# kupc25648/MOP-truss-MARL

Hardware: AMD Instinct MI355X
Metric: env steps/sec (batched FEM solves) at 4096 envs (higher is better)
Workload: dtype f64; 1 GPU; synthetic random-geometry 2-row trusses, 32 nodes / 80 elements / 60 DOF, FEM-only env.step (action decode + FP64 assembly/solve + stresses + point), no agent; envs_per_gpu=4096, global_envs=4096, nodes=32, elements=80, ndof=60, half_bandwidth=7, lanes_per_env=16, rows_per_lane=1, parallelism=env-batch sharded over 1 GPU(s), no data-path collective

## Files before the change

mop-truss-marl_amd/csrc/truss_body.h:

```cpp
#pragma once
#include <stdint.h>
#include <math.h>

#ifndef TB_OPAQUE
#define TB_OPAQUE(x) (x)
#endif
#ifndef TB_SCHED_FENCE
#define TB_SCHED_FENCE()
#endif
#ifndef TRUSS_HD
#error "define TRUSS_HD (e.g. __device__ __forceinline__) before including truss_body.h"
#endif

#define TF_TOP 1
#define TF_RESX 2
#define TF_RESY 4
#define TF_LOAD_BRIDGE 8
#define TF_LOAD_ROOF 16

#define TB_NO_DECODE 0x1u
#define TB_CLAMP_INPLACE 0x2u
#define TB_EMIT_OBS 0x4u

#if defined(__clang__)
typedef uint32_t tb_u4 __attribute__((ext_vector_type(4)));
typedef uint32_t tb_u2 __attribute__((ext_vector_type(2)));
typedef float tb_f4 __attribute__((ext_vector_type(4)));
typedef float tb_f2 __attribute__((ext_vector_type(2)));
typedef double tb_d2 __attribute__((ext_vector_type(2)));
#else
typedef uint32_t tb_u4 __attribute__((vector_size(16)));
typedef uint32_t tb_u2 __attribute__((vector_size(8)));
typedef float tb_f4 __attribute__((vector_size(16)));
typedef float tb_f2 __attribute__((vector_size(8)));
typedef double tb_d2 __attribute__((vector_size(16)));
#endif
TRUSS_HD void tb_ld_row(const double *p, double *dst, int n2) {
  const tb_d2 *q = (const tb_d2 *)__builtin_assume_aligned(p, 16);
  for (int i = 0; i < n2; ++i) {
    tb_d2 v = q[i];
    dst[2 * i] = v[0];
    dst[2 * i + 1] = v[1];
  }
}

struct TopoDev {
  int32_t N, E, NP, ndof, n_pad, n_rest, n_sym_nodes, n_sym_elems, n_sections, has_pairs;
  int32_t nteams, KA, mid, rowsA, rowsB, zlen, dlen, zslot;
  const char *blob;
  int32_t blob_bytes;
  int32_t f_conn;
  int32_t f_pairs;
  int32_t f_nflags;
  int32_t f_dofpos;
  int32_t f_restslot;
  int32_t f_asm;
  int32_t f_diagoff;
  int32_t f_zcode;
  int32_t f_posnode;
  int32_t f_symn;
  int32_t f_syme;
  int32_t f_area;
  int32_t f_isr;
  int32_t f_adj8;
  int32_t f_exs;
  int32_t f_areaf;
  int32_t f_vsf;
  double e_mod, long_stress;
  int32_t o_env0, env_stride;
  int32_t o_kb, o_zs, o_xsol, o_red, o_rbuf, o_par, o_y, o_x, o_tg, o_geo, o_tac, o_sec, o_ev, o_zring, o_mrg;
  int32_t so_q0, so_sr, so_disp, so_mu, so_md, so_comp;
  int32_t emit_ok;
  const char *etab;
  int32_t o_flag;
  int32_t et_xn, et_nxn, et_mat, f_tnxe;
  int32_t nc_xn, nc_nxn, nc_nxe, nc_mat;
  int32_t nxe_cw;
  int32_t b_const;
  int32_t b_erec;
  int32_t b_erec2;
  int32_t b_tc;
  int32_t b_nraw;
  int32_t b_nna, b_nnb, b_nn8;
};

#define TB_TAB(type, base, off) ((const type *)((base) + (off)))

struct StepArgsDev {
  int32_t B;
  uint32_t flags;
  const float *x, *y_in;
  const int32_t *sec_in;
  const float *mu_in, *md_in;
  float *a_geo, *a_topo;
  const uint8_t *coin;
  const float *target;
  const double *env_params;
  float *y_out;
  int32_t *sec_out;
  float *mu_out, *md_out;
  float *disp, *q0, *sr;
  uint8_t *comp;
  float *point, *obj;
  double *disp64, *q064, *energy, *react;
  int32_t *status;
  float *x_n, *A_s, *A_ts, *A_cs, *nxn, *nxe;
};

#define TRUSS_NRED 6

#ifndef TRUSS_BAND_PAD
#define TRUSS_BAND_PAD 1
#endif
constexpr bool tb_band_padded(int G, int WL, int RPL, int EPL, bool emit) {
  return TRUSS_BAND_PAD == 2 ? !emit : TRUSS_BAND_PAD != 0 && !emit && G == 16 && WL == 8 && RPL == 1 && EPL == 5;
}
constexpr int tb_band_stride(int G, int WL, int RPL, int EPL, bool emit) {
  return WL * RPL + (tb_band_padded(G, WL, RPL, EPL, emit) ? 2 : 0);
}
constexpr int tb_band_team_b(int rowsA, int ks, int w) {
  return rowsA * ks + (ks != w ? ((64 - rowsA * ks * 8) & 127) / 8 : 0);
}

TRUSS_HD float tb_clamp01(float v) { return v > 1.0f ? 1.0f : (v < 0.0f ? 0.0f : v); }

TRUSS_HD float tb_round2(float v) { return rintf(v * 100.0f) / 100.0f; }

template <int G, int WL, int RPL, int EPL, bool EMIT = false>
struct StepLane {
  static constexpr int W = WL * RPL;
  static constexpr int KS = tb_band_stride(G, WL, RPL, EPL, EMIT);
  static_assert(KS % 2 == 0, "band rows are read as 16-byte units");
  static constexpr int WL_ = WL;
  static constexpr int G_ = G;
  static constexpr bool EMIT_ = EMIT;
  static constexpr int NPL = (2 * EPL + 4) / 5;
  static constexpr int EPB = 64 / G;
  static constexpr int NDEG = 8;
  static constexpr int NT = G / WL;

  int lane, g, gs, team, env, envc;
  double *Kt, *Zt, *ZRt;
  bool active;
  const char *TB;
  char *L;
  double max_def, load_x, load_y;
  float ymax32, dmin32, ymd32, int1, int2;
  int is_roof;
  double ek[EPL], ec[EPL], es[EPL], ei[EPL];
  double R[RPL][W];
  double rhs[RPL];
  double xs[W];
  int bad;
  double p_vol, p_dt, p_en;
  float p_c1, p_c2;

  TRUSS_HD double *kb(const TopoDev &T) { return (double *)(L + T.o_kb); }
  TRUSS_HD static int team_b(const TopoDev &T) { return tb_band_team_b(T.rowsA, KS, W); }
  TRUSS_HD double *zs(const TopoDev &T) { return (double *)(L + T.o_zs); }
  TRUSS_HD double *xsol(const TopoDev &T) { return (double *)(L + T.o_xsol); }
  TRUSS_HD double *red(const TopoDev &T) { return (double *)(L + T.o_red); }
  TRUSS_HD double *rbuf(const TopoDev &T) { return (double *)(L + T.o_rbuf); }
  TRUSS_HD double *par(const TopoDev &T) { return (double *)(L + T.o_par); }
  TRUSS_HD float *ysh(const TopoDev &T) { return (float *)(L + T.o_y); }
  TRUSS_HD float *xsh(const TopoDev &T) { return (float *)(L + T.o_x); }
  TRUSS_HD float *tgsh(const TopoDev &T) { return (float *)(L + T.o_tg); }
  TRUSS_HD float *geosh(const TopoDev &T) { return (float *)(L + T.o_geo); }
  TRUSS_HD float *tac(const TopoDev &T) { return (float *)(L + T.o_tac); }
  TRUSS_HD int32_t *secsh(const TopoDev &T) { return (int32_t *)(L + T.o_sec); }
  TRUSS_HD int32_t *coinsh(const TopoDev &T) { return (int32_t *)(L + T.env_stride - 4); }
  TRUSS_HD static bool coin_used(const TopoDev &T, const StepArgsDev &A) {
    return T.n_sym_nodes > 0 && !(A.flags & TB_NO_DECODE) && A.coin;
  }
  TRUSS_HD double *evsh(const TopoDev &T) { return (double *)(L + T.o_ev); }
  TRUSS_HD const int16_t *t_conn(const TopoDev &T) const { return TB_TAB(int16_t, TB, T.f_conn); }
  TRUSS_HD const int16_t *t_pairs(const TopoDev &T) const { return TB_TAB(int16_t, TB, T.f_pairs); }
  TRUSS_HD const uint8_t *t_nflags(const TopoDev &T) const { return TB_TAB(uint8_t, TB, T.f_nflags); }
  TRUSS_HD const int16_t *t_dofpos(const TopoDev &T) const { return TB_TAB(int16_t, TB, T.f_dofpos); }
  TRUSS_HD const int16_t *t_restslot(const TopoDev &T) const { return TB_TAB(int16_t, TB, T.f_restslot); }
  TRUSS_HD const int16_t *t_asm(const TopoDev &T) const { return TB_TAB(int16_t, TB, T.f_asm); }
  TRUSS_HD const int16_t *t_diagoff(const TopoDev &T) const { return TB_TAB(int16_t, TB, T.f_diagoff); }
  TRUSS_HD const uint8_t *t_zcode(const TopoDev &T) const { return TB_TAB(uint8_t, TB, T.f_zcode); }
  TRUSS_HD const int16_t *t_posnode(const TopoDev &T) const { return TB_TAB(int16_t, TB, T.f_posnode); }
  TRUSS_HD const int16_t *t_symn(const TopoDev &T) const { return TB_TAB(int16_t, TB, T.f_symn); }
  TRUSS_HD const int16_t *t_syme(const TopoDev &T) const { return TB_TAB(int16_t, TB, T.f_syme); }
  TRUSS_HD const double *t_area(const TopoDev &T) const { return TB_TAB(double, TB, T.f_area); }
  TRUSS_HD const double *t_isr(const TopoDev &T) const { return TB_TAB(double, TB, T.f_isr); }
  TRUSS_HD const int16_t *t_adj8(const TopoDev &T) const { return TB_TAB(int16_t, TB, T.f_adj8); }
  TRUSS_HD const int16_t *t_exs(const TopoDev &T) const { return TB_TAB(int16_t, TB, T.f_exs); }

  TRUSS_HD void init(int lane_, int block, const TopoDev &T, const StepArgsDev &A, char *lds) {
    lane = lane_;
    g = lane % G;
    gs = g % WL;
    team = T.nteams == 2 ? (g / WL) & 1 : 0;
    int grp = lane / G;
    env = block * EPB + grp;
    active = env < A.B;
    envc = active ? env : A.B - 1;
    TB = lds;
    L = lds + T.o_env0 + (size_t)grp * T.env_stride;
    Kt = (double *)(L + T.o_kb) + team * team_b(T);
    Zt = (double *)(L + T.o_zs) + team * T.zlen;
    ZRt = (double *)(L + T.o_zring) + team * W;
    bad = 0;
    p_vol = p_dt = p_en = 0.0;
    p_c1 = p_c2 = 0.0f;
    rs_first_step = 0;
    rs_y_out = A.y_out;
    rs_sec_out = A.sec_out;
    rs_next_geo = rs_next_topo = nullptr;
  }

  static constexpr int BIT = 8;
  static constexpr int BIT_BIG = 20;
  static constexpr int NCAP = (G * ((2 * EPL + 4) / 5) > 64) ? G * ((2 * EPL + 4) / 5) : 64;
  static constexpr int ECAP = (G * EPL > 128) ? G * EPL : 128;
  static constexpr int NIT = (NCAP / 4 + G - 1) / G;
  static constexpr int EIT = (ECAP / 4 + G - 1) / G;
  tb_u4 pg[2 * NIT], pa[3 * NIT];
  int rs_first_step;
  float *rs_y_out;
  int32_t *rs_sec_out;
  const float *rs_next_geo, *rs_next_topo;
  TRUSS_HD void rollout_prefetch(const TopoDev &T, const StepArgsDev &A) {
    if (rs_next_geo) {
      const size_t bn = (size_t)envc * T.N;
      row_load<2 * NIT>(rs_next_geo + bn * 2, 2 * (T.N >> 2), pg);
      row_load<3 * NIT>(rs_next_topo + bn * 3, 3 * (T.N >> 2), pa);
    }
  }
  TRUSS_HD void rollout_stash(const TopoDev &T, const StepArgsDev &A) {
    if (rs_next_geo) {
      row_store<2 * NIT>(geosh(T), 2 * (T.N >> 2), pg);
      row_store<3 * NIT>(tac(T), 3 * (T.N >> 2), pa);
    }
  }

  TRUSS_HD void stage_row_slow(const void *src, void *dst, int nwords) const {
    const uint32_t *s1 = (const uint32_t *)src;
    uint32_t *d1 = (uint32_t *)dst;
    for (int q = g; q < nwords; q += G) d1[q] = s1[q];
  }

  template <int IT>
  TRUSS_HD void row_load(const void *src, int nq, tb_u4 (&v)[IT]) const {
    const tb_u4 *s4 = (const tb_u4 *)src;
#pragma unroll
    for (int i = 0; i < IT; ++i) {
      int q = g + G * i;
      v[i] = s4[q < nq ? q : nq - 1];
    }
  }
  template <int IT>
  TRUSS_HD void row_store(void *dst, int nq, const tb_u4 (&v)[IT]) const {
    tb_u4 *d4 = (tb_u4 *)dst;
#pragma unroll
    for (int i = 0; i < IT; ++i) {
      int q = g + G * i;
      d4[q < nq ? q : nq - 1] = v[i];
    }
  }

  TRUSS_HD void band_clear(const TopoDev &T) {
    tb_u4 *K4 = (tb_u4 *)kb(T);
    const tb_u4 z = {0u, 0u, 0u, 0u};
    const int tot4 = (KS == W ? (T.rowsA + T.rowsB) * W : team_b(T) + T.rowsB * KS) >> 1;
    for (int i = g; i < tot4; i += G) K4[i] = z;
  }

  template <int BI>
  TRUSS_HD void stage_fast(const TopoDev &T, const StepArgsDev &A, bool decode) {
    const size_t bn = (size_t)envc * T.N, be = (size_t)envc * T.E;
    {
      const int nb = T.blob_bytes >> 4, nn = T.N >> 2, ne = T.E >> 2;
      tb_u4 vb[BI], vy[NIT], vx[NIT], vt[NIT], vs[EIT], vp[1], vg[2 * NIT], va[3 * NIT];
      {
        const tb_u4 *s4 = (const tb_u4 *)T.blob;
#pragma unroll
        for (int i = 0; i < BI; ++i) {
          int q = lane + 64 * i;
          vb[i] = s4[q < nb ? q : nb - 1];
        }
      }
      row_load<NIT>(A.y_in + bn, nn, vy);
      row_load<NIT>(A.x + bn, nn, vx);
      row_load<NIT>(A.target + bn, nn, vt);
      row_load<EIT>(A.sec_in + be, ne, vs);
      row_load<1>(A.env_params + (size_t)envc * 8, 4, vp);
      if (decode) {
        row_load<2 * NIT>(A.a_geo + bn * 2, 2 * nn, vg);
        row_load<3 * NIT>(A.a_topo + bn * 3, 3 * nn, va);
      }
      const bool coin = coin_used(T, A);
      int cb = 0;
      if (coin) cb = A.coin[envc];
      band_clear(T);
      {
        tb_u4 *d4 = (tb_u4 *)TB;
#pragma unroll
        for (int i = 0; i < BI; ++i) {
          int q = lane + 64 * i;
          d4[q < nb ? q : nb - 1] = vb[i];
        }
      }
      row_store<NIT>(ysh(T), nn, vy);
      row_store<NIT>(xsh(T), nn, vx);
      row_store<NIT>(tgsh(T), nn, vt);
      row_store<EIT>(secsh(T), ne, vs);
      row_store<1>(par(T), 4, vp);
      if (decode) {
        row_store<2 * NIT>(geosh(T), 2 * nn, vg);
        row_store<3 * NIT>(tac(T), 3 * nn, va);
      }
      if (coin) *coinsh(T) = cb;
    }
  }

  TRUSS_HD void phase_stage(const TopoDev &T, const StepArgsDev &A) {
    const size_t bn = (size_t)envc * T.N, be = (size_t)envc * T.E;
    const bool decode = !(A.flags & TB_NO_DECODE);
    const bool fast = (T.N & 3) == 0 && (T.E & 3) == 0 && T.N <= NCAP && T.E <= ECAP && T.blob_bytes <= BIT_BIG * 64 * 16;
    if (rs_first_step != 0) {
      band_clear(T);
      return;
    }
    if (fast) {
      if (T.blob_bytes <= 3 * 64 * 16) stage_fast<3>(T, A, decode);
      else if (T.blob_bytes <= BIT * 64 * 16) stage_fast<BIT>(T, A, decode);
      else stage_fast<BIT_BIG>(T, A, decode);
    } else {
      const bool coin = coin_used(T, A);
      int cb = 0;
      if (coin) cb = A.coin[envc];
      {
        const tb_u4 *s4 = (const tb_u4 *)T.blob;
        tb_u4 *d4 = (tb_u4 *)TB;
        for (int q = lane; q < (T.blob_bytes >> 4); q += 64) d4[q] = s4[q];
      }
      stage_row_slow(A.y_in + bn, ysh(T), T.N);
      stage_row_slow(A.x + bn, xsh(T), T.N);
      stage_row_slow(A.target + bn, tgsh(T), T.N);
      stage_row_slow(A.sec_in + be, secsh(T), T.E);
      stage_row_slow(A.env_params + (size_t)envc * 8, par(T), 16);
      if (decode) {
        stage_row_slow(A.a_geo + bn * 2, geosh(T), 2 * T.N);
        stage_row_slow(A.a_topo + bn * 3, tac(T), 3 * T.N);
      }
      band_clear(T);
      if (coin) *coinsh(T) = cb;
    }
  }

  TRUSS_HD void load_params(const TopoDev &T) {
    const double *P = par(T);
    double y_max = P[0], d_min = P[1];
    max_def = P[2];
    load_x = P[3];
    load_y = P[4];
    int1 = (float)P[5];
    int2 = (float)P[6];
    is_roof = P[7] != 0.0;
    ymax32 = (float)y_max;
    dmin32 = (float)d_min;
    ymd32 = (float)(y_max - d_min);
  }

  TRUSS_HD void move_range(bool top, float y, float yp, float &up, float &dn) const {
    float upt = fabsf(ymax32 - y), dnt = fabsf((y - yp) - dmin32);
    float upb = is_roof ? fabsf((yp - y) - dmin32) : 0.0f, dnb = is_roof ? fabsf(y) : 0.0f;
    up = top ? upt : upb;
    dn = top ? dnt : dnb;
  }

  TRUSS_HD float move_node(float y, float g0, float g1, float mu, float md, bool resy) const {
    bool down = g1 > g0;
    float a = down ? g1 : g0;
    float rng = down ? md : mu;
    float step = (a * rng) * 0.25f;
    y = down ? (y - step) : (y + step);
    y = tb_round2(y);
    return resy ? 0.0f : y;
  }

  struct PairIn {
    int n0, n1, f0, f1;
    float y0, y1, ga0, ga1, gb0, gb1, ta[3], tb[3];
    float mu0, md0, mu1, md1;
  };
  TRUSS_HD void pair_load(const TopoDev &T, int p, PairIn &q) {
    const float *Y = ysh(T), *GE = geosh(T), *TA = tac(T);
    const int16_t *PR = t_pairs(T);
    const uint8_t *NF = t_nflags(T);
    q.n0 = PR[2 * p];
    q.n1 = PR[2 * p + 1];
    q.y0 = Y[q.n0];
    q.y1 = Y[q.n1];
    q.f0 = NF[q.n0];
    q.f1 = NF[q.n1];
    q.ga0 = GE[2 * q.n0];
    q.ga1 = GE[2 * q.n0 + 1];
    q.gb0 = GE[2 * q.n1];
    q.gb1 = GE[2 * q.n1 + 1];
#pragma unroll
    for (int j = 0; j < 3; ++j) {
      q.ta[j] = TA[3 * q.n0 + j];
      q.tb[j] = TA[3 * q.n1 + j];
    }
  }
  TRUSS_HD void pair_ranges_load(const TopoDev &T, const StepArgsDev &A, PairIn &q) const {
    const size_t bn = (size_t)envc * T.N;
    q.mu0 = A.mu_in[bn + q.n0];
    q.md0 = A.md_in[bn + q.n0];
    q.mu1 = A.mu_in[bn + q.n1];
    q.md1 = A.md_in[bn + q.n1];
  }
  TRUSS_HD void pair_decode(const TopoDev &T, const StepArgsDev &A, PairIn &q, bool real) {
    const size_t bn = (size_t)envc * T.N;
    float *Y = ysh(T), *TA = tac(T);
    const int n0 = q.n0, n1 = q.n1;
    const bool top0 = q.f0 & TF_TOP, top1 = q.f1 & TF_TOP;
    const float ga0 = tb_clamp01(q.ga0), ga1 = tb_clamp01(q.ga1), gb0 = tb_clamp01(q.gb0), gb1 = tb_clamp01(q.gb1);
#pragma unroll
    for (int j = 0; j < 3; ++j) {
      q.ta[j] = tb_clamp01(q.ta[j]);
      q.tb[j] = tb_clamp01(q.tb[j]);
      TA[3 * n0 + j] = q.ta[j];
      TA[3 * n1 + j] = q.tb[j];
    }
    if ((A.flags & TB_CLAMP_INPLACE) && active && real) {
      A.a_geo[(bn + n0) * 2 + 0] = ga0;
      A.a_geo[(bn + n0) * 2 + 1] = ga1;
      A.a_geo[(bn + n1) * 2 + 0] = gb0;
      A.a_geo[(bn + n1) * 2 + 1] = gb1;
#pragma unroll
      for (int j = 0; j < 3; ++j) {
        A.a_topo[(bn + n0) * 3 + j] = q.ta[j];
        A.a_topo[(bn + n1) * 3 + j] = q.tb[j];
      }
    }
    float mu0, md0, mu1, md1;
    if (A.mu_in) {
      mu0 = q.mu0;
      md0 = q.md0;
      mu1 = q.mu1;
      md1 = q.md1;
    } else {
      move_range(top0, q.y0, q.y1, mu0, md0);
      move_range(top1, q.y1, q.y0, mu1, md1);
    }
    float a = move_node(q.y0, ga0, ga1, mu0, md0, q.f0 & TF_RESY);
    float b = move_node(q.y1, gb0, gb1, mu1, md1, q.f1 & TF_RESY);
    const bool c1 = a < 0.0f;
    a = c1 ? (top0 ? dmin32 : 0.0f) : a;
    b = (c1 && top0) ? 0.0f : b;
    const bool c2 = b < 0.0f;
    b = c2 ? (top1 ? dmin32 : 0.0f) : b;
    a = (c2 && top1) ? 0.0f : a;
    const bool c3 = a > ymax32;
    a = c3 ? (top0 ? ymax32 : ymd32) : a;
    b = (c3 && !top0) ? ymax32 : b;
    const bool c4 = b > ymax32;
    b = c4 ? (top1 ? ymax32 : ymd32) : b;
    a = (c4 && !top1) ? ymax32 : a;
    a = (top0 && fabsf(a - b) < dmin32) ? b + dmin32 : a;
    b = (top1 && fabsf(b - a) < dmin32) ? a + dmin32 : b;
    if (real) {
      Y[n0] = a;
      Y[n1] = b;
    }
  }
  TRUSS_HD void phase_decode(const TopoDev &T, const StepArgsDev &A) {
    load_params(T);
    if (A.flags & TB_NO_DECODE) return;
    constexpr int PPL = (NPL + 1) / 2;
    PairIn q[PPL];
#pragma unroll
    for (int i = 0; i < PPL; ++i) {
      const int p = g + G * i;
      pair_load(T, p < T.NP ? p : T.NP - 1, q[i]);
    }
    if (A.mu_in) {
#pragma unroll
      for (int i = 0; i < PPL; ++i) pair_ranges_load(T, A, q[i]);
    }
#pragma unroll
    for (int i = 0; i < PPL; ++i) pair_decode(T, A, q[i], g + G * i < T.NP);
    for (int p = g + G * PPL; p < T.NP; p += G) {
      PairIn r;
      pair_load(T, p, r);
      if (A.mu_in) pair_ranges_load(T, A, r);
      pair_decode(T, A, r, true);
    }
  }

  TRUSS_HD void phase_sym_nodes(const TopoDev &T) {
    float *Y = ysh(T);
    const int16_t *SN = t_symn(T);
    const bool heads = *coinsh(T) != 0;
    for (int i = g; i < T.n_sym_nodes; i += G) {
      int dst = SN[2 * i], src = SN[2 * i + 1];
      float v = heads ? Y[src] : Y[dst];
      Y[dst] = v;
      Y[src] = v;
    }
  }

  TRUSS_HD void phase_sizing(const TopoDev &T, const StepArgsDev &A) {
    if (A.flags & TB_NO_DECODE) return;
    const float *TA = tac(T);
    int32_t *S = secsh(T);
    const int16_t *CN = t_conn(T);
    int n0[EPL], n1[EPL], sc[EPL];
    float a0[EPL][3], a1[EPL][3];
#pragma unroll
    for (int i = 0; i < EPL; ++i) {
      const int e = g + G * i;
      const int ee = e < T.E ? e : T.E - 1;
      const uint32_t c = *(const uint32_t *)(CN + 2 * ee);
      n0[i] = (int)(int16_t)(c & 0xffffu);
      n1[i] = (int)(int16_t)(c >> 16);
      sc[i] = S[ee];
    }
#pragma unroll
    for (int i = 0; i < EPL; ++i) {
#pragma unroll
      for (int j = 0; j < 3; ++j) {
        a0[i][j] = TA[n0[i] * 3 + j];
        a1[i][j] = TA[n1[i] * 3 + j];
      }
    }
#pragma unroll
    for (int i = 0; i < EPL; ++i) {
      const float p0 = a0[i][0] + a1[i][0], p1 = a0[i][1] + a1[i][1], p2 = a0[i][2] + a1[i][2];
      int am = 0;
      float best = p0;
      if (p1 > best) { am = 1; best = p1; }
      if (p2 > best) { am = 2; }
      const int s = sc[i];
      const int sdn = s > 0 ? s - 1 : 0, sup = s < T.n_sections - 1 ? s + 1 : T.n_sections - 1;
      sc[i] = am == 0 ? sdn : (am == 1 ? sup : s);
    }
#pragma unroll
    for (int i = 0; i < EPL; ++i) {
      const int e = g + G * i;
      if (e < T.E) S[e] = sc[i];
    }
  }

  TRUSS_HD void phase_sym_elems(const TopoDev &T) {
    int32_t *S = secsh(T);
    const int16_t *SE = t_syme(T);
    for (int i = g; i < T.n_sym_elems; i += G) {
      int a = SE[2 * i], b = SE[2 * i + 1];
      int m = S[a] < S[b] ? S[a] : S[b];
      S[a] = m;
      S[b] = m;
    }
  }

  TRUSS_HD double load_at(const TopoDev &T, int r) const {
    if (r < 0 || r >= T.ndof) return 0.0;
    int nd = t_posnode(T)[r];
    if (nd < 0) return 0.0;
    int fl = t_nflags(T)[nd >> 1] & (is_roof ? TF_LOAD_ROOF : TF_LOAD_BRIDGE);
    if (!fl) return 0.0;
    return (nd & 1) ? load_y : load_x;
  }
  TRUSS_HD int orig_pos(const TopoDev &T, int tm, int p) const { return tm ? T.ndof - 1 - p : p; }
  TRUSS_HD double team_load(const TopoDev &T, int tm, int p) const {
    if (T.nteams == 1) return load_at(T, p);
    if (tm == 0) return p < T.ndof - T.KA ? load_at(T, p) : 0.0;
    return p < T.KA ? load_at(T, T.ndof - 1 - p) : 0.0;
  }

  static constexpr bool EBATCH = RPL == 1 && W <= 8 && EPL <= 5;
  static constexpr int ECH = EBATCH ? EPL : 1;
  TRUSS_HD void phase_elements(const TopoDev &T, const StepArgsDev &A) {
    const float *Y = ysh(T), *X = xsh(T);
    const int32_t *S = secsh(T);
    const int16_t *CN = t_conn(T);
    const double *AR = t_area(T), *ISR = t_isr(T);
    double *K = kb(T);
    const int16_t *AC = t_asm(T);
    double *EV = evsh(T);
    if (g == 0) EV[3 * T.E] = EV[3 * T.E + 1] = EV[3 * T.E + 2] = 0.0;
#pragma unroll
    for (int c0 = 0; c0 < EPL; c0 += ECH) {
      int n0[ECH], n1[ECH], sc[ECH], ev[ECH];
      tb_u2 code[ECH];
      float x0[ECH], x1[ECH], y0[ECH], y1[ECH];
      double Aa[ECH];
#pragma unroll
      for (int j = 0; j < ECH; ++j) {
        const int i = c0 + j < EPL ? c0 + j : EPL - 1;
        const int e = g + G * i;
        const int ee = e < T.E ? e : T.E - 1;
        const uint32_t c = *(const uint32_t *)(CN + 2 * ee);
        n0[j] = (int)(int16_t)(c & 0xffffu);
        n1[j] = (int)(int16_t)(c >> 16);
        sc[j] = S[ee];
        code[j] = *(const tb_u2 *)(AC + 4 * ee);
        ev[j] = 3 * ee;
      }
#pragma unroll
      for (int j = 0; j < ECH; ++j) {
        x0[j] = X[n0[j]];
        x1[j] = X[n1[j]];
        y0[j] = Y[n0[j]];
        y1[j] = Y[n1[j]];
        Aa[j] = AR[sc[j]];
      }
#pragma unroll
      for (int j = 0; j < ECH; ++j) {
        const int i = c0 + j;
        if (i < EPL) {
          const double dx = (double)x1[j] - (double)x0[j];
          const double dy = (double)y1[j] - (double)y0[j];
          const double l2 = dx * dx + dy * dy;
          const double rl = tb_rsqrt(l2);
          const double len = l2 * rl;
          const double c = dx * rl, s = dy * rl;
// ... 1278 lines not shown
```

mop-truss-marl_amd/csrc/truss_hip.hip:

```cpp
#include <hip/hip_runtime.h>

#include <atomic>
#include <cstdint>
#include <cstdio>
#include <cstring>
#include <type_traits>

#include "../../include/truss_mi355.h"

#pragma clang fp contract(off)

#define TRUSS_HD __device__ __forceinline__
#define TRUSS_UNROLL _Pragma("unroll")
#define TB_SCHED_FENCE() __builtin_amdgcn_sched_barrier(0)
__device__ __forceinline__ int tb_opaque(int x) {
  asm volatile("" : "+v"(x));
  return x;
}
#define TB_OPAQUE(x) tb_opaque(x)
#define TB_STREAM_STORE(p, v) __builtin_nontemporal_store((v), (p))
#ifdef TRUSS_OBS_STORE_NT
#define TB_OBS_STORE(p, v) __builtin_nontemporal_store((v), (p))
#else
#define TB_OBS_STORE(p, v) (*(p) = (v))
#endif

__device__ __forceinline__ void tb_lds_add(double *p, double v) { unsafeAtomicAdd(p, v); }

template <int WL, int SRC>
__device__ __forceinline__ double tb_dpp_bcast(double v) {
#ifndef TRUSS_BCAST32
  if constexpr (WL == 16 || WL == 8) {
    const long long b = __double_as_longlong(v);
    long long r;
    if constexpr (WL == 16) {
      r = __builtin_amdgcn_update_dpp(0ll, b, 0x150 + SRC, 0xf, 0xf, false);
    } else {
      r = __builtin_amdgcn_update_dpp(0ll, b, 0x150 + SRC, 0xf, 0x3, false);
      r = __builtin_amdgcn_update_dpp(r, b, 0x150 + 8 + SRC, 0xf, 0xc, false);
    }
    return __longlong_as_double(r);
  }
#endif
  const int lo = __double2loint(v), hi = __double2hiint(v);
  int rlo, rhi;
  if constexpr (WL == 16) {
    rlo = __builtin_amdgcn_update_dpp(lo, lo, 0x150 + SRC, 0xf, 0xf, false);
    rhi = __builtin_amdgcn_update_dpp(hi, hi, 0x150 + SRC, 0xf, 0xf, false);
  } else if constexpr (WL == 8) {
    rlo = __builtin_amdgcn_update_dpp(lo, lo, 0x150 + SRC, 0xf, 0x3, false);
    rlo = __builtin_amdgcn_update_dpp(rlo, lo, 0x150 + 8 + SRC, 0xf, 0xc, false);
    rhi = __builtin_amdgcn_update_dpp(hi, hi, 0x150 + SRC, 0xf, 0x3, false);
    rhi = __builtin_amdgcn_update_dpp(rhi, hi, 0x150 + 8 + SRC, 0xf, 0xc, false);
  } else {
    static_assert(WL == 4, "team width");
    constexpr int qp = SRC | (SRC << 2) | (SRC << 4) | (SRC << 6);
    rlo = __builtin_amdgcn_update_dpp(lo, lo, qp, 0xf, 0xf, false);
    rhi = __builtin_amdgcn_update_dpp(hi, hi, qp, 0xf, 0xf, false);
  }
  return __hiloint2double(rhi, rlo);
}
template <class LN>
__device__ __forceinline__ double tb_team_bcast(LN &ln, int src) {
  constexpr int WL = LN::WL_;
  switch (src) {
#define TB_CASE(i) \
  case i:          \
    if constexpr (i < WL) return tb_dpp_bcast<WL, i>(ln.bx); else break;
    TB_CASE(0) TB_CASE(1) TB_CASE(2) TB_CASE(3) TB_CASE(4) TB_CASE(5) TB_CASE(6) TB_CASE(7)
    TB_CASE(8) TB_CASE(9) TB_CASE(10) TB_CASE(11) TB_CASE(12) TB_CASE(13) TB_CASE(14) TB_CASE(15)
#undef TB_CASE
  }
  return ln.bx;
}

__device__ __forceinline__ double tb_rcp(double d) {
  double r = __builtin_amdgcn_rcp(d);
  r = fma(fma(-d, r, 1.0), r, r);
  r = fma(fma(-d, r, 1.0), r, r);
  return r;
}

__device__ __forceinline__ float tb_rcpf(float d) {
  float r = __builtin_amdgcn_rcpf(d);
  return fmaf(fmaf(-d, r, 1.0f), r, r);
}

#ifdef TRUSS_STOP_AT
#define TRUSS_ST(i) do { if ((i) == TRUSS_STOP_AT) return; } while (0)
#endif
#ifdef TRUSS_STAMPS
__device__ unsigned long long g_truss_stamps[32];
__device__ unsigned long long g_truss_span[4096][6];
#define TRUSS_ST(i)                                                  \
  do {                                                               \
    __builtin_amdgcn_sched_barrier(0);                               \
    if (threadIdx.x == 0 && blockIdx.x == gridDim.x / 2) g_truss_stamps[i] = clock64(); \
    if (threadIdx.x == 0 && ((i) == 0 || (i) == 9) && blockIdx.x < 4096) {              \
      g_truss_span[blockIdx.x][(i) == 0 ? 0 : 2] = clock64();                            \
      g_truss_span[blockIdx.x][(i) == 0 ? 1 : 3] = wall_clock64();                       \
    }                                                                \
    __builtin_amdgcn_sched_barrier(0);                               \
  } while (0)
#endif

__device__ __forceinline__ double tb_rsqrt(double x) {
  double r = __builtin_amdgcn_rsq(x);
  r = r * fma(-0.5 * x, r * r, 1.5);
  r = r * fma(-0.5 * x, r * r, 1.5);
  return r;
}

template <int G, bool MAX>
__device__ __forceinline__ float tb_group_reduce(float v) {
  auto op = [](float a, float b) { return MAX ? fmaxf(a, b) : fminf(a, b); };
  auto dpp = [](float x, auto ctrl) {
    return __int_as_float(__builtin_amdgcn_update_dpp(0, __float_as_int(x), decltype(ctrl)::value, 0xf, 0xf, false));
  };
  if constexpr (G >= 2) v = op(v, dpp(v, std::integral_constant<int, 0xB1>{}));
  if constexpr (G >= 4) v = op(v, dpp(v, std::integral_constant<int, 0x4E>{}));
  if constexpr (G >= 8) v = op(v, dpp(v, std::integral_constant<int, 0x141>{}));
  if constexpr (G >= 16) v = op(v, dpp(v, std::integral_constant<int, 0x140>{}));
  if constexpr (G >= 32) v = op(v, __shfl_xor(v, 16));
  if constexpr (G >= 64) v = op(v, __shfl_xor(v, 32));
  return v;
}
template <class LN>
__device__ __forceinline__ float tb_group_min(LN &ln, int c) { return tb_group_reduce<LN::G_, false>(ln.pmn[c]); }
template <class LN>
__device__ __forceinline__ float tb_group_max(LN &ln, int c) { return tb_group_reduce<LN::G_, true>(ln.pmx[c]); }

template <int G>
__device__ __forceinline__ double tb_group_reduce_sum(double v) {
  auto dpp = [](double x, auto ctrl) {
    const int lo = __builtin_amdgcn_update_dpp(0, __double2loint(x), decltype(ctrl)::value, 0xf, 0xf, false);
    const int hi = __builtin_amdgcn_update_dpp(0, __double2hiint(x), decltype(ctrl)::value, 0xf, 0xf, false);
    return __hiloint2double(hi, lo);
  };
  if constexpr (G >= 2) v = v + dpp(v, std::integral_constant<int, 0xB1>{});
  if constexpr (G >= 4) v = v + dpp(v, std::integral_constant<int, 0x4E>{});
  if constexpr (G >= 8) v = v + dpp(v, std::integral_constant<int, 0x141>{});
  if constexpr (G >= 16) v = v + dpp(v, std::integral_constant<int, 0x140>{});
  if constexpr (G >= 32) v = v + __shfl_xor(v, 16);
  if constexpr (G >= 64) v = v + __shfl_xor(v, 32);
  return v;
}
template <class LN>
__device__ __forceinline__ double tb_group_sum_d(LN &ln, int which) {
  return tb_group_reduce_sum<LN::G_>(which == 0 ? ln.p_vol : which == 1 ? ln.p_dt : ln.p_en);
}
template <class LN>
__device__ __forceinline__ float tb_group_max_f(LN &ln, int which) {
  return tb_group_reduce<LN::G_, true>(which == 0 ? ln.p_c1 : which == 1 ? ln.p_c2 : (float)ln.bad);
}

template <class LN, class TD>
__device__ __forceinline__ bool tb_obs_timed_out(LN &ln, const TD &T) {
  if constexpr (LN::EMIT_) return *((const __attribute__((address_space(3))) int *)(ln.TB + T.o_flag) + 1) != 0;
  return false;
}

#include "truss_body.h"

typedef __attribute__((address_space(3))) int tb_lds_word;
__device__ __forceinline__ tb_lds_word *tb_flag_ptr(char *lds, int o_flag) { return (tb_lds_word *)(lds + o_flag); }
__device__ __forceinline__ void tb_publish(char *lds, int o_flag, int k) {
  __builtin_amdgcn_wave_barrier();
#ifdef TRUSS_FLAG_RELAXED
  __builtin_amdgcn_fence(__ATOMIC_RELEASE, "wavefront");
  if (threadIdx.x == 0) __hip_atomic_store(tb_flag_ptr(lds, o_flag), k, __ATOMIC_RELAXED, __HIP_MEMORY_SCOPE_WORKGROUP);
#else
  if (threadIdx.x == 0) __hip_atomic_store(tb_flag_ptr(lds, o_flag), k, __ATOMIC_RELEASE, __HIP_MEMORY_SCOPE_WORKGROUP);
#endif
}
#ifndef TB_AWAIT_SPINS
#define TB_AWAIT_SPINS (1 << 22)
#endif
__device__ __forceinline__ bool tb_await(char *lds, int o_flag, int k) {
  for (int spin = 0; spin < TB_AWAIT_SPINS; ++spin) {
    const int v = __hip_atomic_load(tb_flag_ptr(lds, o_flag), __ATOMIC_ACQUIRE, __HIP_MEMORY_SCOPE_WORKGROUP);
    if (__builtin_amdgcn_readfirstlane(v) >= k) return true;
    __builtin_amdgcn_s_sleep(1);
  }
  return false;
}

template <class LN>
__device__ __forceinline__ void tb_obs_timeout(LN &ln, char *lds, int o_flag, int32_t *status) {
  if ((threadIdx.x & 63) == 0) *(tb_flag_ptr(lds, o_flag) + 1) = 1;
  if (ln.g == 0 && ln.active && status) atomicOr(&status[ln.env], TRUSS_STATUS_OBS_TIMEOUT);
}

#define TB_WAVE_SYNC()                                    \
  do {                                                    \
    __builtin_amdgcn_fence(__ATOMIC_RELEASE, "wavefront"); \
    __builtin_amdgcn_wave_barrier();                      \
    __builtin_amdgcn_fence(__ATOMIC_ACQUIRE, "wavefront"); \
  } while (0)
#define PH(call) \
  ln.call;       \
  TB_WAVE_SYNC()
#define PH_NS(call) ln.call
#define BAR() TB_WAVE_SYNC()

template <int G, int WL, int RPL, int EPL, bool EMIT>
__global__ __launch_bounds__(EMIT ? 128 : 64) void truss_step_kernel(const TopoDev T, const StepArgsDev A) {
  extern __shared__ __attribute__((aligned(16))) char smem[];
  StepLane<G, WL, RPL, EPL, EMIT> ln;
  ln.init(threadIdx.x & 63, blockIdx.x, T, A, smem);
  constexpr int W_ = StepLane<G, WL, RPL, EPL, EMIT>::W;
  constexpr bool EMIT_ = EMIT;
  if constexpr (EMIT) {
    if (threadIdx.x == 0) {
      *tb_flag_ptr(smem, T.o_flag) = 0;
      *(tb_flag_ptr(smem, T.o_flag) + 1) = 0;
    }
    __syncthreads();
    if (threadIdx.x >= 64) {
#ifdef TRUSS_STAMPS
#define SST(i)                                                                                        \
  do {                                                                                                \
    __builtin_amdgcn_sched_barrier(0);                                                                \
    if (threadIdx.x == 64 && blockIdx.x == gridDim.x / 2) g_truss_stamps[i] = clock64();              \
    if (threadIdx.x == 64 && ((i) == 20 || (i) == 26) && blockIdx.x < 4096)                           \
      g_truss_span[blockIdx.x][(i) == 20 ? 4 : 5] = wall_clock64();                                   \
    __builtin_amdgcn_sched_barrier(0);                                                                \
  } while (0)
#else
#define SST(i)
#endif
      ln.emit_tables_load(T);
      __builtin_amdgcn_s_waitcnt(0);
      bool ok = tb_await(smem, T.o_flag, 1);
      if (ok) {
        SST(20);
        TRUSS_STREAM_SEG1(PH, T, A)
        SST(21);
        ok = tb_await(smem, T.o_flag, 2);
      }
      if (ok) {
        SST(22);
        TRUSS_STREAM_SEG2(PH, T, A)
        SST(23);
        ok = tb_await(smem, T.o_flag, 3);
      }
      if (ok) {
        SST(24);
        TRUSS_STREAM_SEG3(PH, T, A)
        SST(25);
      } else {
        tb_obs_timeout(ln, smem, T.o_flag, A.status);
      }
#ifdef TRUSS_STAMPS
      __builtin_amdgcn_s_waitcnt(0);
      SST(26);
#endif
#undef SST
      return;
    }
  }
#ifdef TRUSS_FAULT_DROP_PUBLISH3
#define EMIT_POINT(k) do { if ((k) != 3) tb_publish(smem, T.o_flag, k); } while (0)
#else
#define EMIT_POINT(k) tb_publish(smem, T.o_flag, k)
#endif
  TRUSS_STEP_SCHEDULE(PH, PH_NS, BAR, T, A)
#undef EMIT_POINT
}

struct RolloutDev {
  TopoDev T;
  StepArgsDev A;
  int32_t n_steps, n_sets;
  size_t gstride, tstride;
};
template <int G, int WL, int RPL, int EPL>
__global__ __launch_bounds__(64) void truss_rollout_kernel(const RolloutDev P_) {
  extern __shared__ __attribute__((aligned(16))) char smem[];
  constexpr int W_ = StepLane<G, WL, RPL, EPL, false>::W;
  constexpr bool EMIT_ = false;
#define EMIT_POINT(k) (void)0
  const int n_steps = P_.n_steps;
  for (int s = 0; s < n_steps; ++s) {
    typedef const char __attribute__((address_space(4))) *tb_kernarg_ptr;
    tb_kernarg_ptr ka = (tb_kernarg_ptr)__builtin_amdgcn_kernarg_segment_ptr();
    asm volatile("" : "+s"(ka));
    const RolloutDev &P = *(const RolloutDev *)ka;
    const TopoDev &T = P.T;
    const StepArgsDev &A = P.A;
    StepLane<G, WL, RPL, EPL, false> ln;
    int lane_id = threadIdx.x;
    asm volatile("" : "+v"(lane_id));
    ln.init(lane_id, blockIdx.x, T, A, smem);
    const int nset = (s + 1) % P.n_sets;
    ln.rs_first_step = s;
    ln.rs_y_out = (s & 1) ? (float *)A.y_in : A.y_out;
    ln.rs_sec_out = (s & 1) ? (int32_t *)A.sec_in : A.sec_out;
    ln.rs_next_geo = s + 1 < n_steps ? A.a_geo + (size_t)nset * P.gstride : nullptr;
    ln.rs_next_topo = s + 1 < n_steps ? A.a_topo + (size_t)nset * P.tstride : nullptr;
    TRUSS_STEP_SCHEDULE(PH, PH_NS, BAR, T, A)
    TB_WAVE_SYNC();
  }
#undef EMIT_POINT
}

#undef PH
#undef PH_NS
#undef BAR
#undef TB_WAVE_SYNC

__global__ __launch_bounds__(64) void truss_obs_kernel(const TopoDev T, const ObsArgsDev A) {
  extern __shared__ __attribute__((aligned(16))) char smem[];
  ObsLane ln;
  ln.init(threadIdx.x, blockIdx.x, blockIdx.y, T, A, smem);
#define PH(call) \
  ln.call;       \
  __syncthreads()
#define PH_NS(call) ln.call
  const int r0_tile = ln.role == 1 ? ((int)blockIdx.y - 1) * A.tile_rows : 0;
  TRUSS_OBS_SCHEDULE(PH, PH_NS, T, A, r0_tile)
#undef PH
#undef PH_NS
}

#define TRUSS_BACKEND_NAME "hip"
struct truss_topo;
static void *tb_dev_alloc(size_t n) {
  void *p = nullptr;
  return hipMalloc(&p, n) == hipSuccess ? p : nullptr;
}
static void tb_dev_free(void *p) { (void)hipFree(p); }
static bool tb_dev_upload(void *dst, const void *src, size_t n) {
  return hipMemcpy(dst, src, n, hipMemcpyHostToDevice) == hipSuccess;
}
static int tb_launch_step(const truss_topo *t, const StepArgsDev &A, bool emit, void *stream);
static int tb_launch_obs(const truss_topo *t, const ObsArgsDev &A, void *stream);
static int tb_launch_rollout(const truss_topo *t, const StepArgsDev &A, int n_steps, int n_sets, void *stream);

#include "truss_host.h"

static constexpr int TB_MAX_DEVICES = 64;
struct TbLdsOptIn {
  std::atomic<bool> done[TB_MAX_DEVICES];
  int ensure(const void *kern) {
    int dev = 0;
    if (hipGetDevice(&dev) != hipSuccess || dev < 0 || dev >= TB_MAX_DEVICES) return tb_fail(TRUSS_EHIP, "hipGetDevice failed");
    if (done[dev].load(std::memory_order_acquire)) return TRUSS_OK;
    if (hipFuncSetAttribute(kern, hipFuncAttributeMaxDynamicSharedMemorySize, 160 * 1024) != hipSuccess)
      return tb_fail(TRUSS_EHIP, "hipFuncSetAttribute(MaxDynamicSharedMemorySize) failed");
    done[dev].store(true, std::memory_order_release);
    return TRUSS_OK;
  }
};
static int tb_launched(const char *what) {
  const hipError_t e = hipGetLastError();
  return e == hipSuccess ? TRUSS_OK : tb_fail(TRUSS_EHIP, std::string(what) + hipGetErrorString(e));
}

static int tb_launch_obs(const truss_topo *t, const ObsArgsDev &A, void *stream) {
  static TbLdsOptIn optin;
  if (int rc = optin.ensure((const void *)truss_obs_kernel)) return rc;
  hipLaunchKernelGGL(truss_obs_kernel, dim3((unsigned)A.B, (unsigned)(A.n_split > 1 ? A.n_split + 1 : 1)), dim3(64), tb_obs_lds_bytes(t->N), (hipStream_t)stream, t->dev, A);
  return tb_launched("obs kernel launch failed: ");
}

template <int G, int WL, int RPL, int EPL, bool EMIT>
static int hip_run(const truss_topo *t, const StepArgsDev &A, hipStream_t st) {
  static TbLdsOptIn optin;
  auto kern = truss_step_kernel<G, WL, RPL, EPL, EMIT>;
  if (int rc = optin.ensure((const void *)kern)) return rc;
  constexpr int EPB = 64 / G;
  const unsigned grid = (unsigned)((A.B + EPB - 1) / EPB);
  hipLaunchKernelGGL(kern, dim3(grid), dim3(EMIT ? 128 : 64), EMIT ? t->lds_bytes_emit : t->lds_bytes, st, EMIT ? t->dev_emit : t->dev, A);
  return tb_launched("kernel launch failed: ");
}

template <int G, int WL, int RPL, int EPL>
static int hip_run_rollout(const truss_topo *t, const StepArgsDev &A, int n_steps, int n_sets, hipStream_t st) {
  static TbLdsOptIn optin;
  auto kern = truss_rollout_kernel<G, WL, RPL, EPL>;
  if (int rc = optin.ensure((const void *)kern)) return rc;
  RolloutDev Q;
  Q.T = t->dev;
  Q.A = A;
  Q.n_steps = n_steps;
  Q.n_sets = n_sets;
  Q.gstride = (size_t)A.B * t->N * 2;
  Q.tstride = (size_t)A.B * t->N * 3;
  constexpr int EPB = 64 / G;
  const unsigned grid = (unsigned)((A.B + EPB - 1) / EPB);
  hipLaunchKernelGGL(kern, dim3(grid), dim3(64), t->lds_bytes, st, Q);
  return tb_launched("rollout kernel launch failed: ");
}
static int tb_launch_rollout(const truss_topo *t, const StepArgsDev &A, int n_steps, int n_sets, void *stream) {
  const TbVariant &v = kVariants[t->variant];
#define X(g, wl, r, e) \
  if (v.G == g && v.WL == wl && v.RPL == r && v.EPL == e) return hip_run_rollout<g, wl, r, e>(t, A, n_steps, n_sets, (hipStream_t)stream);
  TRUSS_ROLLOUT_VARIANTS(X)
#undef X
  return tb_fail(TRUSS_EUNSUPPORTED, "variant not compiled with the persistent rollout");
}

static int tb_launch_step(const truss_topo *t, const StepArgsDev &A, bool emit, void *stream) {
  const TbVariant &v = kVariants[t->variant];
  hipStream_t st = (hipStream_t)stream;
  if (emit) {
#define X(g, wl, r, e) \
  if (v.G == g && v.WL == wl && v.RPL == r && v.EPL == e) return hip_run<g, wl, r, e, true>(t, A, st);
    TRUSS_EMIT_VARIANTS(X)
#undef X
    return tb_fail(TRUSS_EUNSUPPORTED, "variant not compiled with the observation writer");
  }
#define X(g, wl, r, e) \
  if (v.G == g && v.WL == wl && v.RPL == r && v.EPL == e) return hip_run<g, wl, r, e, false>(t, A, st);
  TRUSS_VARIANTS(X)
#undef X
  return tb_fail(TRUSS_EUNSUPPORTED, "variant not compiled");
}

#ifdef TRUSS_STAMPS
extern "C" int truss_debug_span(unsigned long long *out, int nblocks) {
  return hipMemcpyFromSymbol(out, HIP_SYMBOL(g_truss_span), (size_t)nblocks * 6 * sizeof(unsigned long long)) == hipSuccess ? 0 : -3;
}
extern "C" int truss_debug_stamps32(unsigned long long *out32) {
  return hipMemcpyFromSymbol(out32, HIP_SYMBOL(g_truss_stamps), 32 * sizeof(unsigned long long)) == hipSuccess ? 0 : -3;
}
extern "C" int truss_debug_stamps(unsigned long long *out16) {
  return hipMemcpyFromSymbol(out16, HIP_SYMBOL(g_truss_stamps), 16 * sizeof(unsigned long long)) == hipSuccess ? 0 : -3;
}
#endif

#include "truss_gcn.h"
#include "truss_gcn_group.h"
#include "truss_gcn_level.h"
#include "truss_gcn_level_bwd.h"
#include "truss_replay.h"

#include "truss_front.h"
#include "truss_reward.h"
#include "truss_archive.h"
#include "truss_pairs.h"
#include "truss_gcn_aggregate.h"
#include "truss_gcn_level_agg.h"
#include "truss_optim.h"
#include "truss_critic_tail.h"
```

Measured before the change: 242.6 million env-steps/s.

## Issue stage global loads before init and reload kernargs to overlap latency

For the G=16/WL=8/RPL=1/EPL=5 configuration, the kernel now issues the per-env global loads (blob, y, x, target, sections, params, actions, coin) into registers at the very start, before lane init and the EMIT sync. The later phase_stage clears the band and stores those registers to LDS instead of loading them then. Kernel arguments are re-read from the kernarg segment so the scalar loads are pinned early. This hides global-memory latency behind setup work, at the cost of higher register pressure and more fragile, layout-dependent kernarg access.

```diff
diff --git a/mop-truss-marl_amd/csrc/truss_body.h b/mop-truss-marl_amd/csrc/truss_body.h
--- a/mop-truss-marl_amd/csrc/truss_body.h
+++ b/mop-truss-marl_amd/csrc/truss_body.h
@@ -7,6 +7,9 @@
 #endif
 #ifndef TB_SCHED_FENCE
 #define TB_SCHED_FENCE()
+#endif
+#ifndef TB_ARGS_FIRST
+#define TB_ARGS_FIRST(...)
 #endif
 #ifndef TRUSS_HD
 #error "define TRUSS_HD (e.g. __device__ __forceinline__) before including truss_body.h"
@@ -270,6 +273,57 @@
   }
 
   template <int BI>
+  struct StageRegs {
+    tb_u4 vb[BI], vy[NIT], vx[NIT], vt[NIT], vs[EIT], vp[1], vg[2 * NIT], va[3 * NIT];
+    int cb;
+  };
+  template <int BI>
+  TRUSS_HD void stage_fast_load(const TopoDev &T, const StepArgsDev &A, bool decode, StageRegs<BI> &r) const {
+    const size_t bn = (size_t)envc * T.N, be = (size_t)envc * T.E;
+    const int nb = T.blob_bytes >> 4, nn = T.N >> 2, ne = T.E >> 2;
+    {
+      const tb_u4 *s4 = (const tb_u4 *)T.blob;
+#pragma unroll
+      for (int i = 0; i < BI; ++i) {
+        int q = lane + 64 * i;
+        r.vb[i] = s4[q < nb ? q : nb - 1];
+      }
+    }
+    row_load<NIT>(A.y_in + bn, nn, r.vy);
+    row_load<NIT>(A.x + bn, nn, r.vx);
+    row_load<NIT>(A.target + bn, nn, r.vt);
+    row_load<EIT>(A.sec_in + be, ne, r.vs);
+    row_load<1>(A.env_params + (size_t)envc * 8, 4, r.vp);
+    if (decode) {
+      row_load<2 * NIT>(A.a_geo + bn * 2, 2 * nn, r.vg);
+      row_load<3 * NIT>(A.a_topo + bn * 3, 3 * nn, r.va);
+    }
+    r.cb = 0;
+    if (coin_used(T, A)) r.cb = A.coin[envc];
+  }
+  template <int BI>
+  TRUSS_HD void stage_fast_store(const TopoDev &T, const StepArgsDev &A, bool decode, const StageRegs<BI> &r) {
+    const int nb = T.blob_bytes >> 4, nn = T.N >> 2, ne = T.E >> 2;
+    {
+      tb_u4 *d4 = (tb_u4 *)TB;
+#pragma unroll
+      for (int i = 0; i < BI; ++i) {
+        int q = lane + 64 * i;
+        d4[q < nb ? q : nb - 1] = r.vb[i];
+      }
+    }
+    row_store<NIT>(ysh(T), nn, r.vy);
+    row_store<NIT>(xsh(T), nn, r.vx);
+    row_store<NIT>(tgsh(T), nn, r.vt);
+    row_store<EIT>(secsh(T), ne, r.vs);
+    row_store<1>(par(T), 4, r.vp);
+    if (decode) {
+      row_store<2 * NIT>(geosh(T), 2 * nn, r.vg);
+      row_store<3 * NIT>(tac(T), 3 * nn, r.va);
+    }
+    if (coin_used(T, A)) *coinsh(T) = r.cb;
+  }
+  template <int BI>
   TRUSS_HD void stage_fast(const TopoDev &T, const StepArgsDev &A, bool decode) {
     const size_t bn = (size_t)envc * T.N, be = (size_t)envc * T.E;
     {
@@ -316,8 +370,43 @@
       if (coin) *coinsh(T) = cb;
     }
   }
+  TRUSS_HD static bool stage_is_fast(const TopoDev &T) {
+    return (T.N & 3) == 0 && (T.E & 3) == 0 && T.N <= NCAP && T.E <= ECAP && T.blob_bytes <= BIT_BIG * 64 * 16;
+  }
+
+  static constexpr bool PRE = G == 16 && WL == 8 && RPL == 1 && EPL == 5;
+  static constexpr int PRE_BI = 3;
+  StageRegs<PRE_BI> pre_r;
+  int pre_issued = 0;
+  TRUSS_HD void stage_issue(int lane_, int block, const TopoDev &T, const StepArgsDev &A) {
+    if constexpr (!PRE) return;
+    TB_ARGS_FIRST(T.N, T.E, T.blob_bytes, T.n_sym_nodes, A.B, A.flags, T.blob, A.y_in, A.x, A.target, A.sec_in, A.env_params, A.a_geo,
+                  A.a_topo, A.coin, T.o_env0, T.env_stride, T.o_kb, T.o_zs, T.rowsA, T.rowsB, T.o_par, T.emit_ok, A.mu_out, A.disp64,
+                  A.nxe);
+    lane = lane_;
+    g = lane % G;
+    const int e = block * EPB + lane / G;
+    envc = e < A.B ? e : A.B - 1;
+    if (stage_is_fast(T) && T.blob_bytes <= PRE_BI * 64 * 16) {
+      stage_fast_load<PRE_BI>(T, A, !(A.flags & TB_NO_DECODE), pre_r);
+      pre_issued = 1;
+    }
+  }
+
+  TRUSS_HD static void stage_args_second(const TopoDev &T, const StepArgsDev &A) {
+    if constexpr (!PRE) return;
+    TB_ARGS_FIRST(T.N, T.E, T.blob_bytes, T.n_sym_nodes, T.nteams, T.rowsA, T.rowsB, T.zlen, T.o_env0, T.env_stride, T.o_kb, T.o_zs,
+                  T.o_zring, T.o_par, T.o_y, T.o_x, T.o_tg, T.o_geo, T.o_tac, T.o_sec, A.B, A.flags, A.coin, A.y_out, A.sec_out);
+  }
 
   TRUSS_HD void phase_stage(const TopoDev &T, const StepArgsDev &A) {
+    if constexpr (PRE) {
+      if (pre_issued) {
+        band_clear(T);
+        stage_fast_store<PRE_BI>(T, A, !(A.flags & TB_NO_DECODE), pre_r);
+        return;
+      }
+    }
     const size_t bn = (size_t)envc * T.N, be = (size_t)envc * T.E;
     const bool decode = !(A.flags & TB_NO_DECODE);
     const bool fast = (T.N & 3) == 0 && (T.E & 3) == 0 && T.N <= NCAP && T.E <= ECAP && T.blob_bytes <= BIT_BIG * 64 * 16;
diff --git a/mop-truss-marl_amd/csrc/truss_hip.hip b/mop-truss-marl_amd/csrc/truss_hip.hip
--- a/mop-truss-marl_amd/csrc/truss_hip.hip
+++ b/mop-truss-marl_amd/csrc/truss_hip.hip
@@ -18,6 +18,23 @@
   return x;
 }
 #define TB_OPAQUE(x) tb_opaque(x)
+template <class V>
+__device__ __forceinline__ void tb_pin_scalar(V v) {
+  asm volatile("" : : "s"(v));
+}
+template <class... Vs>
+__device__ __forceinline__ void tb_args_first(Vs... v) {
+  TB_SCHED_FENCE();
+  (tb_pin_scalar(v), ...);
+  TB_SCHED_FENCE();
+}
+#define TB_ARGS_FIRST(...) tb_args_first(__VA_ARGS__)
+typedef const char __attribute__((address_space(4))) *tb_kernarg_ptr;
+__device__ __forceinline__ tb_kernarg_ptr tb_kernargs_here() {
+  tb_kernarg_ptr ka = (tb_kernarg_ptr)__builtin_amdgcn_kernarg_segment_ptr();
+  asm volatile("" : "+s"(ka) : : "memory");
+  return ka;
+}
 #define TB_STREAM_STORE(p, v) __builtin_nontemporal_store((v), (p))
 #ifdef TRUSS_OBS_STORE_NT
 #define TB_OBS_STORE(p, v) __builtin_nontemporal_store((v), (p))
@@ -204,9 +221,20 @@
 #define BAR() TB_WAVE_SYNC()
 
 template <int G, int WL, int RPL, int EPL, bool EMIT>
-__global__ __launch_bounds__(EMIT ? 128 : 64) void truss_step_kernel(const TopoDev T, const StepArgsDev A) {
+__global__ __launch_bounds__(EMIT ? 128 : 64) void truss_step_kernel(const TopoDev T_, const StepArgsDev A_) {
   extern __shared__ __attribute__((aligned(16))) char smem[];
   StepLane<G, WL, RPL, EPL, EMIT> ln;
+  if (!EMIT || __builtin_amdgcn_readfirstlane(threadIdx.x) < 64) ln.stage_issue(threadIdx.x & 63, blockIdx.x, T_, A_);
+  TB_SCHED_FENCE();
+  struct Kernargs { TopoDev T; StepArgsDev A; };
+  constexpr size_t a_off = (sizeof(TopoDev) + 7) & ~(size_t)7;
+  static_assert(alignof(StepArgsDev) == 8 && alignof(TopoDev) == 8 && offsetof(Kernargs, A) == a_off, "kernel-argument layout");
+  constexpr bool PRE = StepLane<G, WL, RPL, EPL, EMIT>::PRE;
+  tb_kernarg_ptr ka = nullptr;
+  if constexpr (PRE) ka = tb_kernargs_here();
+  const TopoDev &T = [&]() -> const TopoDev & { if constexpr (PRE) return *(const TopoDev *)ka; else return T_; }();
+  const StepArgsDev &A = [&]() -> const StepArgsDev & { if constexpr (PRE) return *(const StepArgsDev *)(ka + a_off); else return A_; }();
+  ln.stage_args_second(T, A);
   ln.init(threadIdx.x & 63, blockIdx.x, T, A, smem);
   constexpr int W_ = StepLane<G, WL, RPL, EPL, EMIT>::W;
   constexpr bool EMIT_ = EMIT;
```

Measured after the change: 247.3 million env-steps/s (median of 6 runs). 1.9% higher.
